# k-flouris/cmf

Hardware: AMD Instinct MI355X
Metric: log-density evals/sec (JtJ-cholesky path), MNIST D=784 d=64 bs=512 (higher is better)
Workload: dtype f32 (3x3 tangent convs as bf16x3 split MFMA, fp32 accumulate); 1 GPU; C3: MNIST-shaped (1,28,28) uint8-range + U[0,1) noise, non-square flow d=64, cholesky J^T J log-det + g_ij off-diagonal L1 + reconstruction, eval/no_grad; per_gpu_batch=512, global_batch=512, D=784, latent_dimension=64, parallelism=dp1

## Files before the change

### cmf_amd/_lib.py

```python
import ctypes as C
import os
import threading

_HERE = os.path.dirname(os.path.abspath(__file__))
LIB_PATH = os.path.join(_HERE, "libcmf_amd.so")

F_NONE, F_RELU, F_TANH, F_RAW, F_SELF_RELU, F_RELU_BITS = 0, 1, 2, 3, 4, 5
O_NONE, O_TANH, O_STANH = 0, 1, 2
GRAM_INVALID, GRAM_RING64, GRAM_DIRECT128, GRAM_WIDE, GRAM_RING_LIMIT = 0, 64, 128, 512, 0x7fffff00

_fp = C.c_void_p
_ll = C.c_longlong
_i = C.c_int
_f = C.c_float
_d = C.c_double


class ConvTangentArgs(C.Structure):
    _fields_ = [("x", _fp), ("x_np", _ll), ("x_ci", _ll), ("x_px", _ll),
                ("f", _fp), ("f_np", _ll), ("f_ci", _ll), ("f_px", _ll), ("fmode", _i),
                ("w", _fp),
                ("y", _fp), ("y_np", _ll), ("y_co", _ll), ("y_px", _ll),
                ("r", _fp), ("r_np", _ll), ("r_co", _ll), ("r_px", _ll),
                ("np", _i), ("cin", _i), ("cout", _i), ("H", _i), ("W", _i), ("nc", _i), ("taps", _i),
                ("bias", _fp), ("f_group", _i), ("x_sl", _ll), ("y_sl", _ll), ("r_sl", _ll),
                ("fo", _fp), ("fo_np", _ll), ("fo_co", _ll), ("fo_px", _ll), ("fomode", _i),
                ("mask_out", _fp), ("mask_np", _ll), ("amax_in", _fp), ("amax_out", _fp), ("live", _i),
                ("ymask", _fp), ("ymask_np", _ll),
                ("head_w", _fp), ("head_cout", _i), ("head_a", _fp), ("head_a_np", _ll), ("head_a_c", _ll), ("head_a_px", _ll),
                ("head_y", _fp), ("head_y_np", _ll), ("head_y_co", _ll), ("head_y_px", _ll),
                ("seed", _fp), ("seed_np", _ll), ("seed_col", _ll), ("seed_w", _fp),
                ("block_w1", _fp), ("block_m1", _fp), ("block_m1_np", _ll)]


class ConvPrimalArgs(C.Structure):
    _fields_ = [("x", _fp), ("x_b", _ll), ("x_c", _ll), ("x_px", _ll),
                ("f", _fp), ("f_c", _ll), ("f_px", _ll), ("imode", _i),
                ("w", _fp), ("bias", _fp), ("sw", _fp), ("sb", _fp),
                ("y", _fp), ("y_b", _ll), ("y_c", _ll), ("y_px", _ll),
                ("g", _fp),
                ("r", _fp), ("r_b", _ll), ("r_c", _ll), ("r_px", _ll),
                ("omode", _i),
                ("B", _i), ("cin", _i), ("cout", _i), ("H", _i), ("W", _i), ("taps", _i)]


class ProbeApplyArgs(C.Structure):
    _fields_ = [("r", _fp), ("r_np", _ll), ("r_px", _ll),
                ("t", _fp), ("t_np", _ll), ("t_c", _ll), ("t_px", _ll),
                ("cls", _fp),
                ("y", _fp), ("y_np", _ll), ("y_px", _ll),
                ("ymask", _fp), ("ymask_np", _ll),
                ("np", _i), ("cin", _i), ("H", _i), ("W", _i), ("nc", _i), ("ns", _i)]


MLP_MAX_LAYERS = 8
WGRAD_MAX_BATCH = 16


class MlpCouplerArgs(C.Structure):
    _fields_ = [("z", _fp), ("z_b", _ll), ("t", _fp), ("t_f", _ll), ("w", _fp),
                ("zi", _fp), ("si", _fp), ("ti", _fp), ("n_mod", _i),
                ("B", _i), ("cin", _i), ("chan_off", _i), ("chan_step", _i), ("n_layers", _i),
                ("width", _i * (MLP_MAX_LAYERS + 1)), ("w_off", _ll * MLP_MAX_LAYERS), ("decode", _i), ("lj", _fp), ("ncols", _i)]


SIGNATURES = {
    "cmf_version": (C.c_char_p, []),
    "cmf_pack_weight": (_i, [_fp, _fp, _i, _i, _i, _i, C.POINTER(_ll), _fp]),
    "cmf_pack_weights_batched": (_i, [_fp, _i, _fp]),
    "cmf_conv_tangent": (_i, [C.POINTER(ConvTangentArgs), _fp]),
    "cmf_pack_weight_bf16x3": (_i, [_fp, _fp, _i, _i, C.POINTER(_ll), _fp]),
    "cmf_pack_weight_bf16x3_t": (_i, [_fp, _fp, _i, _i, _i, C.POINTER(_ll), _fp]),
    "cmf_conv_tangent_bf16x3": (_i, [C.POINTER(ConvTangentArgs), _fp]),
    "cmf_probe_apply": (_i, [C.POINTER(ProbeApplyArgs), _fp]),
    "cmf_pack_seed_weight": (_i, [_fp, _fp, _fp]),
    "cmf_seed_panel": (_i, [_fp, _ll, _ll, _fp, _fp, _ll, _ll, _i, _i, _i, _i, _fp]),
    "cmf_pack_block_weight": (_i, [_fp, _fp, C.POINTER(_ll), _fp]),
    "cmf_pack_weight_f16x3": (_i, [_fp, _fp, _i, _i, _i, C.POINTER(_ll), _fp]),
    "cmf_conv_tangent_f16x3": (_i, [C.POINTER(ConvTangentArgs), _fp]),
    "cmf_conv_tangent_f16x3_item": (_i, [C.POINTER(ConvTangentArgs), _i, _fp]),
    "cmf_absmax": (_i, [_fp, _ll, _fp, _fp]),
    "cmf_conv_tangent_wgrad_ws": (_ll, [C.POINTER(ConvTangentArgs)]),
    "cmf_conv_tangent_wgrad": (_i, [C.POINTER(ConvTangentArgs), _fp, _fp, _fp, _ll, _fp]),
    "cmf_conv_tangent_wgrad_bf16x3": (_i, [C.POINTER(ConvTangentArgs), _fp, _fp, _fp, _ll, _fp]),
    "cmf_conv_tangent_wgrad_bf16x3_batched": (_i, [C.POINTER(ConvTangentArgs), _i, C.POINTER(_fp), C.POINTER(_fp), C.POINTER(_fp), _fp, _ll, _fp]),
    "cmf_primal_regroup": (_i, [_fp, _fp, _i, _ll, _i, _fp]),
    "cmf_conv_primal": (_i, [C.POINTER(ConvPrimalArgs), _fp]),
    "cmf_acl_primal": (_i, [_fp, _ll, _fp, _ll, _fp, _fp, _fp, _i, _i, _i, _fp, _fp]),
    "cmf_acl_tangent": (_i, [_fp, _ll, _ll, _fp, _ll, _ll, _i, _fp, _ll, _fp, _ll, _fp, _fp, _fp, _fp, _i, _i, _fp]),
    "cmf_acl_cotangent": (_i, [_fp, _ll, _ll, _fp, _ll, _ll, _i, _fp, _ll, _fp, _ll, _fp, _fp, _fp, _fp, _i, _i, _fp]),
    "cmf_acl_primal_backward": (_i, [_fp, _ll, _fp, _ll, _fp, _ll, _fp, _fp, _fp, _fp, _i, _i, _i, _fp, _fp]),
    "cmf_acl_cross_terms": (_i, [_fp, _ll, _ll, _fp, _ll, _ll, _fp, _ll, _ll, _i, _fp, _ll, _fp, _ll, _fp, _fp, _fp, _fp, _i, _i,
                            _fp, _fp, _fp, _fp]),
    "cmf_gather_primal": (_i, [_fp, _ll, _fp, _ll, _fp, _i, _i, _fp]),
    "cmf_gather_tangent": (_i, [_fp, _ll, _ll, _fp, _ll, _ll, _fp, _i, _i, _i, _fp]),
    "cmf_seed_tangent": (_i, [_fp, _ll, _ll, _fp, _i, _i, _fp, _i, _i, _i, _fp]),
    "cmf_gram_cholesky": (_i, [_fp, _ll, _ll, _i, _i, _i, _i, _fp, _fp, _fp, _fp, _fp, _fp, _fp]),
    "cmf_cholesky_retry": (_i, [_fp, _i, _i, _i, _f, _fp, _fp, _fp, _fp, _fp]),
    "cmf_gram_cholesky_family": (_i, [_i, _i, _ll]),
    "cmf_gram_condition": (_i, [_fp, _fp, _i, _i, _f, _fp, _fp, _fp, _fp, _fp]),
    "cmf_metric_stats_ws": (_ll, [_i, _i, _i, _i]),
    "cmf_metric_stats_accumulate": (_i, [_fp, _i, _i, _i, _fp, _fp, _ll, _fp, _fp]),
    "cmf_gram_spectrum": (_i, [_fp, _i, _i, _fp, _fp, _fp, _fp, _fp]),
    "cmf_gauss_newton_step": (_i, [_fp, _ll, _ll, _i, _i, _i, _i, _fp, _fp, _fp, _fp, _fp, _fp, _fp, _fp, _fp]),
    "cmf_weighted_gauss_newton_step": (_i, [_fp, _ll, _ll, _i, _i, _i, _i, _fp, _fp, _fp, _fp, _fp, _fp, _fp, _fp, _fp, _fp]),
    "cmf_operator_apply": (_i, [_fp, _i, _i, _fp, _ll, _ll, _i, _i, _fp, _fp, _ll, _ll, _fp, _fp]),
    "cmf_cross_gram": (_i, [_fp, _ll, _ll, _i, _i, _i, _i, _i, _fp, _fp]),
    "cmf_curve_step_ws": (_ll, [_i, _i, _i]),
    "cmf_curve_step": (_i, [_fp, _ll, _ll, _i, _i, _i, _i, _i, _fp, _fp, _fp, _fp, _fp, _fp, _fp, _fp, _fp, _fp, _ll, _fp]),
    "cmf_metric_solve": (_i, [_fp, _fp, _i, _i, _i, _fp, _fp, _fp, _fp, _fp]),
# ... 133 lines not shown
```

### cmf_amd/csrc/conv_block_head.hip

```cpp
#include <stdint.h>

#include "common.h"

namespace {

typedef __bf16 bf16x8 __attribute__((ext_vector_type(8)));
typedef __bf16 bf16x2 __attribute__((ext_vector_type(2)));
typedef float f32x2 __attribute__((ext_vector_type(2)));
typedef unsigned u32x4 __attribute__((ext_vector_type(4)));

constexpr int HID = 64, KJ = HID * 9, NT = 512, ROWS = 16, ND = 25, HALO = 8, XB = 4;
constexpr int SLICE = HID * 16;
static_assert(2 * KJ > 2 * NT && 2 * KJ <= 3 * NT && (2 * KJ - 2 * NT) % 64 == 0, "phase B: two units per thread, a third for whole waves");
constexpr int W1_FRAGS = 9 * 4 * 2 * 2 * 64;

__device__ __forceinline__ unsigned pack_hi(float a, float b, float& ra, float& rb) {
  bf16x2 h = __builtin_convertvector(f32x2{a, b}, bf16x2);
  const unsigned bits = __builtin_bit_cast(unsigned, h);
  ra = a - __builtin_bit_cast(float, bits << 16);
  rb = b - __builtin_bit_cast(float, bits & 0xffff0000u);
  return bits;
}
__device__ __forceinline__ unsigned pack_lo(float a, float b) {
  bf16x2 h = __builtin_convertvector(f32x2{a, b}, bf16x2);
  return __builtin_bit_cast(unsigned, h);
}

__global__ void pack_block_weight_kernel(const float* __restrict__ w, u32x4* __restrict__ out) {
  const int idx = blockIdx.x * 256 + threadIdx.x;
  if (idx >= W1_FRAGS) return;
  const int l = idx & 63, hl = (idx >> 6) & 1, ks = (idx >> 7) & 1, ct = (idx >> 8) & 3, t1 = idx >> 10;
  const int c = 16 * ct + (l & 15), ci0 = 32 * ks + 8 * (l >> 4);
  unsigned r[4];
#pragma unroll
  for (int jj = 0; jj < 4; ++jj) {
    const float v0 = w[((ci0 + 2 * jj) * HID + c) * 9 + t1], v1 = w[((ci0 + 2 * jj + 1) * HID + c) * 9 + t1];
    float ra, rb;
    const unsigned h = pack_hi(v0, v1, ra, rb);
    r[jj] = hl ? pack_lo(ra, rb) : h;
  }
  out[idx] = u32x4{r[0], r[1], r[2], r[3]};
}

struct Tile {
  int row0, s0, xb, Ws, H, W, live;
  __device__ __forceinline__ bool slot(int p, int& row, int& col, int& po) const {
    const int s = s0 + (p & 1);
    row = row0 + (p >> 1);
    col = live ? 2 * s + ((row + live - 1) & 1) : s;
    po = row * Ws + s;
    return row < H && s < Ws;
  }
};

__device__ __forceinline__ void load_w1(u32x4 (&b)[2][2], const u32x4* __restrict__ wp, int ct, int lane, int t1) {
#pragma unroll
  for (int ks = 0; ks < 2; ++ks)
#pragma unroll
    for (int hl = 0; hl < 2; ++hl) b[ks][hl] = wp[(((t1 * 4 + ct) * 2 + ks) * 2 + hl) * 64 + lane];
}

template <int HALF, int CP>
__device__ __forceinline__ void build_half(const u32x4* __restrict__ wp, const u32x4* As, float* Ks, const float* Gs,
                                           const unsigned long long* ha, const int* ctr, int ct, int lane) {
  constexpr int D0 = HALF ? 12 : 0, NDH = HALF ? 13 : 12;
  const f32x4 zero = {0.f, 0.f, 0.f, 0.f};
  f32x4 acc[NDH];
  u32x4 af[9][2][2], bw[2][2][2];
#pragma unroll
  for (int i = 0; i < NDH; ++i) acc[i] = zero;
  load_w1(bw[0], wp, ct, lane, 0);
#pragma unroll
  for (int t2 = 0; t2 < 9; ++t2)
#pragma unroll
    for (int ks = 0; ks < 2; ++ks)
#pragma unroll
      for (int hl = 0; hl < 2; ++hl) af[t2][ks][hl] = As[((t2 * 2 + ks) * 2 + hl) * 64 + lane];
#pragma unroll
  for (int t1 = 0; t1 < 9; ++t1) {
    if (t1 < 8) load_w1(bw[(t1 + 1) & 1], wp, ct, lane, t1 + 1);
#pragma unroll
    for (int t2 = 0; t2 < 9; ++t2) {
      const int d = (t1 / 3 + t2 / 3) * 5 + t1 % 3 + t2 % 3;
      if (d >= D0 && d < D0 + NDH) {
#pragma unroll
        for (int ks = 0; ks < 2; ++ks) {
          const bf16x8 ah = __builtin_bit_cast(bf16x8, af[t2][ks][0]), al = __builtin_bit_cast(bf16x8, af[t2][ks][1]);
          const bf16x8 bh = __builtin_bit_cast(bf16x8, bw[t1 & 1][ks][0]), bl = __builtin_bit_cast(bf16x8, bw[t1 & 1][ks][1]);
          acc[d - D0] = __builtin_amdgcn_mfma_f32_16x16x32_bf16(al, bh, acc[d - D0], 0, 0, 0);
          acc[d - D0] = __builtin_amdgcn_mfma_f32_16x16x32_bf16(ah, bl, acc[d - D0], 0, 0, 0);
          acc[d - D0] = __builtin_amdgcn_mfma_f32_16x16x32_bf16(ah, bh, acc[d - D0], 0, 0, 0);
        }
// ... 233 lines not shown
          if (o < cout && (N >= 16 || !(lane & 4))) yb[(long long)o * a.head_y_co + (idx & 3)] = val[i];
        }
      }
    }
  }
}

template <int CP>
int launch(const cmf_conv_tangent_args& a, hipStream_t s) {
  constexpr int P = ROWS / CP, TR = P / 2;
  const int Ws = a.live ? a.W / 2 : a.W;
  const long long tiles_x = (Ws + 1) / 2, tiles = tiles_x * ((a.H + TR - 1) / TR), ntiles = tiles * a.np;
  if (ntiles > 0x7ffffff0LL) return CMF_ERANGE;
  const int grid = 8 * (int)((ntiles + 7) / 8);
  hipLaunchKernelGGL(conv_block_head_kernel<CP>, dim3(grid), dim3(NT), 0, s, a, (int)tiles_x, (int)tiles, (int)ntiles);
  CMF_LAUNCH_CHECK();
  return 0;
}

}

extern "C" int cmf_pack_block_weight(const float* w, void* out, long long* out_bytes, void* stream) {
  if (!out) {
    if (!out_bytes) return CMF_EINVAL;
    *out_bytes = (long long)W1_FRAGS * 16;
    return 0;
  }
  if (!w || (uintptr_t)out % 16 || (uintptr_t)w % 4) return CMF_EINVAL;
  hipLaunchKernelGGL(pack_block_weight_kernel, dim3((W1_FRAGS + 255) / 256), dim3(256), 0, (hipStream_t)stream, w, (u32x4*)out);
  CMF_LAUNCH_CHECK();
  return 0;
}

int cmf_conv_block_head(const cmf_conv_tangent_args& a, hipStream_t s) {
  if (!a.x || !a.w || !a.f || !a.block_w1 || !a.block_m1 || !a.head_w || !a.head_a || !a.head_y) return CMF_EINVAL;
  if (a.r && a.r != a.x) return CMF_EINVAL;
  if (a.fmode != CMF_F_RELU_BITS || a.taps != 9 || a.cin != HID || a.cout != HID) return CMF_EINVAL;
  if (a.head_cout < 1 || a.head_cout > 8 || a.np <= 0 || a.H <= 0 || a.W <= 0 || a.nc <= 0 || a.nc % 16) return CMF_EINVAL;
  if (a.bias || a.fo || a.ymask || a.mask_out || a.seed || a.live < 0 || a.live > 2 || (a.live && a.W % 2)) return CMF_EINVAL;
  if (!((a.W % 14 == 0 && a.H % 2 == 0) || (a.W % 8 == 0 && a.H % 4 == 0))) return CMF_EINVAL;
  const long long HW = (long long)a.H * a.W;
  if (HW > (1 << 24)) return CMF_ERANGE;
  if (a.x_ci != 16 || a.x_sl != SLICE) return CMF_EINVAL;
  if ((a.x_np | a.x_px | a.head_y_np | a.head_y_co | a.head_y_px) % 4) return CMF_EINVAL;
  if (a.x_px < (long long)HID * a.nc || a.head_y_px < a.nc) return CMF_EINVAL;
  if ((uintptr_t)a.x % 16 || (uintptr_t)a.head_y % 16 || (uintptr_t)a.w % 4 || (uintptr_t)a.head_w % 4 || (uintptr_t)a.block_w1 % 16)
    return CMF_EINVAL;
  if ((uintptr_t)a.f % 8 || a.f_np % 8 || a.f_np < HW * (HID / 8)) return CMF_EINVAL;
  if ((uintptr_t)a.block_m1 % 8 || a.block_m1_np % 8 || a.block_m1_np < HW * (HID / 8)) return CMF_EINVAL;
  const int cp = a.head_cout <= 2 ? 2 : a.head_cout <= 4 ? 4 : 8;
  return cp == 2 ? launch<2>(a, s) : cp == 4 ? launch<4>(a, s) : launch<8>(a, s);
}
```

### cmf_amd/engine.py

```python
import ctypes as C
import threading
from typing import NamedTuple

import numpy as np
import torch
import torch.nn as nn

from . import _lib
from ._lib import (F_NONE, F_RELU, F_TANH, F_RAW, F_SELF_RELU, F_RELU_BITS, O_NONE, O_TANH, O_STANH, ConvPrimalArgs,
                   ConvTangentArgs)


def _stream():
    return C.c_void_p(torch.cuda.current_stream().cuda_stream)


def _p(t):
    return None if t is None else C.c_void_p(t.data_ptr())


def require_gpu(t, what="input"):
    if not t.is_cuda:
        raise RuntimeError(f"cmf_amd: {what} is on {t.device}; the log-density path runs only through the HIP "
                           "kernels on an AMD GPU (there is no CPU fallback)")
# ... 360 lines not shown
        run = launch

        def launch():
            with _lib.role("primal"):
                run()

    def cost():
        px_in = float(H) * W * nc * np_
        px = px_in * (0.5 if live else 1.0)
        return (2.0 * (cin + (1 if seed is not None else 0)) * cout * taps * px,
                4.0 * (px_in * cin + px * (cout + (cout if res_t is not None else 0))
                       + (float(seed["np"]) * np_ if seed is not None else 0.0)))
    return _timed(f"conv_tangent_t{taps}_ci{cin}_co{cout}" + ("_primal" if fmode == F_SELF_RELU else "_primal_bwd" if pbwd else "_live" if live else ""),
                  cost, launch)


def _conv_tangent_head(lib, a, x_t, x_off, x_np, x_ci, x_px, weight, taps, y_t, y_np, y_co, y_px, np_, cin, cout, H, W, nc, fmode, f,
                       f_np, res_t, res_off, res_np, x_sl, y_off, live, head):
    wf, act = head["weight"], head["act"]
    hc = int(wf.shape[0])
    w2, wf = weight.detach(), wf.detach().reshape(hc, -1)
    assert w2.is_contiguous() and wf.is_contiguous() and act.is_contiguous() and w2.dtype == wf.dtype == act.dtype == torch.float32
    a.x = C.c_void_p(x_t.data_ptr() + 4 * int(x_off)); a.x_np, a.x_ci, a.x_px, a.x_sl = int(x_np), int(x_ci), int(x_px), int(x_sl)
    a.f = _p(f); a.f_np = int(f_np); a.fmode = int(fmode)
    a.w = _p(w2)
    a.r = None if res_t is None else C.c_void_p(res_t.data_ptr() + 4 * int(res_off))
    a.r_np, a.r_co, a.r_px, a.r_sl = int(x_np if res_np is None else res_np), int(x_ci), int(x_px), int(x_sl)
    a.np, a.cin, a.cout, a.H, a.W, a.nc, a.taps, a.live = int(np_), int(cin), int(cout), int(H), int(W), int(nc), int(taps), int(live)
    blk = head.get("conv1")
    if blk is not None:
        assert res_t is None and isinstance(blk["mask"], BitMask), "the folded block reads h as x and takes relu'(c1) from a BitMask"
        a.block_w1 = _p(_block_pack(blk["weight"], x_t.device))
        a.block_m1, a.block_m1_np = _p(blk["mask"].data), int(blk["mask"].np_bytes)
    a.head_w, a.head_cout = _p(wf), hc
    a.head_a = _p(act); a.head_a_np, a.head_a_c, a.head_a_px = int(cin) * H * W, H * W, 1
    a.head_y = C.c_void_p(y_t.data_ptr() + 4 * int(y_off)); a.head_y_np, a.head_y_co, a.head_y_px = int(y_np), int(y_co), int(y_px)
    launch = lambda: _lib.check(lib.cmf_conv_tangent_bf16x3(C.byref(a), _stream()), "cmf_conv_tangent_bf16x3")

    def cost():
        px_out = float(H) * W * np_ * (0.5 if live else 1.0)
        if blk is not None:
            return (2.0 * hc * px_out * (cin * taps * cout + 3 * taps * cin * taps * cout + 25 * cout * nc),
                    4.0 * (float(H) * W * np_ * (nc * cin + 4) + px_out * (cout + nc * hc)))
        return (2.0 * hc * px_out * (cin * taps * cout + (cin * taps + cout) * nc),
                4.0 * (float(H) * W * np_ * nc * cin + px_out * (nc * cout + cout + nc * hc)))
    return _timed(f"conv_tangent_t{taps}_ci{cin}_co{cout}" + ("_live" if live else ""), cost, launch)


_WGRAD_WS = {}


def conv_tangent_wgrad(x_t, x_off, x_np, x_ci, x_px, gy_t, gy_off, y_np, y_co, y_px, dw, taps, np_, cin, cout, H, W, nc,
                       fmode=F_NONE, f=None, f_np=0, f_ci=0, f_px=0, f_group=1, x_sl=16, y_sl=16, precision=None):
    lib = _lib.load()
    assert dw.dtype == torch.float32 and dw.is_contiguous() and dw.numel() == cout * cin * taps
    a = ConvTangentArgs()
    a.x = C.c_void_p(x_t.data_ptr() + 4 * int(x_off)); a.x_np, a.x_ci, a.x_px = int(x_np), int(x_ci), int(x_px)
    fbits = isinstance(f, BitMask)
    if fbits:
        f, f_np, f_ci, f_px, fmode = f.data, f.np_bytes, 0, 0, F_RELU_BITS
    a.f = _p(f); a.f_np, a.f_ci, a.f_px = int(f_np), int(f_ci), int(f_px); a.fmode = fmode
    a.y_np, a.y_co, a.y_px = int(y_np), int(y_co), int(y_px)
    a.np, a.cin, a.cout, a.H, a.W, a.nc, a.taps = int(np_), int(cin), int(cout), int(H), int(W), int(nc), int(taps)
    a.f_group = int(f_group)
    a.x_sl, a.y_sl = int(x_sl), int(y_sl)
    need = int(lib.cmf_conv_tangent_wgrad_ws(C.byref(a)))
    key = (x_t.device, torch.cuda.current_stream().cuda_stream)
    ws = _WGRAD_WS.get(key)
    if ws is None or ws.numel() * 4 < need:
        ws = _WGRAD_WS[key] = torch.empty(need // 4, dtype=torch.float32, device=x_t.device)
# ... 1317 lines not shown
    y = primal_regroup(yg.view(G, -1), False).view(B, cout, H, W)
    g = primal_regroup(gg.view(G, -1), False).view(B, cout, H, W)
    if not need_acts:
        return y, g, None
    std_of = lambda t: primal_regroup(t.view(G, -1), False).view(B, hid, H, W)
    if train:
        out = ActList([a0] + masks[:-1] + [std_of(acts[-1])] if bits else [a0] + [std_of(t) for t in acts[1:]])
        out.grouped = acts
        return y, g, out
    if bits:
        return y, g, [a0] + masks[:-1] + [std_of(acts[-1])]
    return y, g, [a0] + [std_of(t) for t in acts[1:]]


def _view_rows(T, view):
    if T.layout == "panel":
        HW = view.geom.HW
        rows = T.data[: T.B * T.N * T.nc].view(T.B, T.N // HW, HW * T.nc)[:, view.chan_off::view.chan_step][:, :view.cin]
        out = Tangent(T.B, view.cin * HW, T.nc, "panel", T.data.device)
    else:
        rows = T.data[: T.B * T.N * T.nc].view(T.N, T.B * T.nc)[view.chan_off::view.chan_step][:view.cin]
        out = Tangent(T.B, view.cin, T.nc, "fmajor", T.data.device)
    out.data.view(rows.shape).copy_(rows)
    return out


CHECKERBOARD_TAIL = True
SKIP_DEAD_ROWS = True
FOLD_HEAD = True
FOLD_BLOCK = True
PROBE_FRONT = True
SEED_RESIDUAL = True
FOLD_BLOCK_SHAPES = ((28, 28, 2),)
PROBE_FRONT_SHAPES = {(28, 28, 1)}
PROBE_CLASSES = 13


def probe_plan(mask):
    mask = np.asarray(mask)
    if mask.ndim != 3:
        return None
    cin, H, W = mask.shape
    if not 1 <= cin <= 2:
        return None
    r, col = np.meshgrid(np.arange(H), np.arange(W), indexing="ij")
    cls = (np.mod(r - 5 * col, 2 * PROBE_CLASSES) >> 1)[None] + PROBE_CLASSES * np.arange(cin)[:, None, None]
    cls = np.where(mask != 0, cls, -1).astype(np.int8)
    for r0 in range(H):
        for c0 in range(W):
            win = cls[:, max(r0 - 2, 0):r0 + 3, max(c0 - 2, 0):c0 + 3].reshape(-1)
            win = win[win >= 0]
            if len(np.unique(win)) != len(win):
                return None
    ns = (PROBE_CLASSES * cin + 15) // 16
    flat = cls.reshape(-1)
    probes = np.zeros((cin * H * W, 16 * ns), dtype=np.float32)
    rows = np.flatnonzero(flat >= 0)
    probes[rows, flat[rows]] = 1.0
    return {"cls": flat, "ns": ns, "probes": probes}


def probe_apply(R, r_np, r_px, T, t_off, t_np, t_c, t_px, cls, y, y_np, y_px, np_, cin, H, W, nc, ns, ymask=None):
    a = _lib.ProbeApplyArgs()
    a.r = _p(R); a.r_np, a.r_px = int(r_np), int(r_px)
    a.t = C.c_void_p(T.data_ptr() + 4 * int(t_off)); a.t_np, a.t_c, a.t_px = int(t_np), int(t_c), int(t_px)
    a.cls = _p(cls)
# ... 32 lines not shown
            out[:, 16 * kq:16 * kq + 16, j] = w[:, 3 * kq + j].reshape(4, 16)
    return out


def seed_panel_index(H, W):
    idx = np.full(seed_plane(H, W), -1, dtype=np.int64)
    r, c = np.meshgrid(np.arange(H), np.arange(W), indexing="ij")
    idx[((r + 1) * (W + 2) + c + 1).reshape(-1)] = (r * W + c).reshape(-1)
    return idx


def _seed_pack(conv0, dev):
    def build():
        w = conv0.weight.detach().contiguous()
        assert tuple(w.shape) == (64, 1, 3, 3) and w.dtype == torch.float32
        out = torch.empty(4096, dtype=torch.uint8, device=dev)
        _lib.check(_lib.load().cmf_pack_seed_weight(_p(w), _p(out), _stream()), "cmf_pack_seed_weight")
        return out

    return DERIVED.get((id(conv0.weight), "seed-residual", str(dev)), [conv0.weight], build)


def _block_pack(weight, dev):
    def build():
        w = weight.detach().contiguous()
        assert tuple(w.shape) == (64, 64, 3, 3) and w.dtype == torch.float32
        n = C.c_longlong(0)
        _lib.check(_lib.load().cmf_pack_block_weight(None, None, C.byref(n), None), "pack size")
        out = torch.empty(n.value, dtype=torch.uint8, device=dev)
        _lib.check(_lib.load().cmf_pack_block_weight(_p(w), _p(out), None, _stream()), "cmf_pack_block_weight")
        return out

    return DERIVED.get((id(weight), "fold-block", str(dev)), [weight], build)


def _probe_hidden(conv0, view, plan, H, W, hid, dev):
    HW, ncp = H * W, 16 * plan["ns"]

    def build():
        out = torch.empty(HW * hid * ncp, dtype=torch.float32, device=dev)
        conv_tangent(plan["probes"], 0, view.cin * HW * ncp, HW * ncp, ncp, conv0.weight, 9, out, hid * HW * ncp, 16, hid * ncp,
                     1, view.cin, hid, H, W, ncp, fmode=F_RAW, f=view.mask, f_np=0, f_ci=HW, f_px=1, y_sl=hid * 16)
        return out

    return DERIVED.get((id(conv0.weight), "probe-front", H, W, view.cin, str(dev)), [conv0.weight], build)


def probe_front(conv0, conv1, T, view, plan, factor, ymask, scratch, u, H, W):
    B, nc, HW, hid, dev = T.B, T.nc, H * W, conv1.out_channels, T.data.device
    assert hid == 64 and T.layout == "panel"
    ncp = 16 * plan["ns"]
    conv_tangent(_probe_hidden(conv0, view, plan, H, W, hid, dev), 0, 0, 16, hid * ncp, conv1.weight, 9, scratch,
                 hid * HW * ncp, 16, hid * ncp, B, hid, hid, H, W, ncp, x_sl=hid * 16, y_sl=hid * 16, ymask=ymask, **factor)
    probe_apply(scratch, hid * HW * ncp, hid * ncp, T.data, view.chan_off * HW * nc, T.t_b, view.chan_step * HW * nc, nc,
                plan["cls"], u, hid * HW * nc, hid * nc, B, view.cin, H, W, nc, plan["ns"], ymask=ymask)


class TangentPlan(NamedTuple):
    filt: bool
    front: str
    tail: str
    compact: bool


def resnet_tangent_plan(net, view, nc, layout, acts, training):
    conv0, blocks, convf = _resnet_parts(net)
# ... 340 lines not shown
```

### include/cmf_amd.h

```cpp
#ifndef CMF_AMD_H
#define CMF_AMD_H

#ifdef __cplusplus
extern "C" {
#endif

#define CMF_EINVAL (-1)
#define CMF_ERANGE (-2)

#define CMF_F_NONE 0
#define CMF_F_RELU 1
#define CMF_F_TANH 2
#define CMF_F_RAW  3
#define CMF_F_SELF_RELU 4
#define CMF_F_RELU_BITS 5

#define CMF_O_NONE  0
#define CMF_O_TANH  1
#define CMF_O_STANH 2

const char* cmf_version(void);

int cmf_pack_weight(const float* w, float* out, int cout, int cin, int taps, int transpose,
                    long long* out_floats, void* stream);

typedef struct {
  const float* w; void* out; long long total;
  int cout, cin, taps, transpose, kind, reserved;
} cmf_pack_desc;
int cmf_pack_weights_batched(const cmf_pack_desc* table, int n, void* stream);

typedef struct {
  const float* x; long long x_np, x_ci, x_px;
  const float* f; long long f_np, f_ci, f_px;
  int fmode;
  const float* w;
  float* y;       long long y_np, y_co, y_px;
  const float* r; long long r_np, r_co, r_px;
  int np, cin, cout, H, W, nc, taps;
  const float* bias;
  int f_group;
  long long x_sl, y_sl, r_sl;
  const float* fo; long long fo_np, fo_co, fo_px; int fomode;
  void* mask_out; long long mask_np;
  const float* amax_in; float* amax_out;
  int live;
  const void* ymask; long long ymask_np;
  const float* head_w; int head_cout;
  const float* head_a; long long head_a_np, head_a_c, head_a_px;
  float* head_y; long long head_y_np, head_y_co, head_y_px;
  const float* seed; long long seed_np, seed_col; const void* seed_w;
  const void* block_w1; const void* block_m1; long long block_m1_np;
} cmf_conv_tangent_args;
int cmf_conv_tangent(const cmf_conv_tangent_args* a, void* stream);

int cmf_pack_weight_bf16x3(const float* w, void* out, int cout, int cin, long long* out_bytes, void* stream);
int cmf_pack_weight_bf16x3_t(const float* w, void* out, int cout, int cin, int transpose, long long* out_bytes, void* stream);
int cmf_conv_tangent_bf16x3(const cmf_conv_tangent_args* a, void* stream);
int cmf_pack_seed_weight(const float* w, void* out, void* stream);
int cmf_pack_block_weight(const float* w, void* out, long long* out_bytes, void* stream);
int cmf_seed_panel(const float* v, long long v_np, long long v_px, const float* mask, float* out, long long out_np, long long out_col,
                   int np, int H, int W, int nc, void* stream);

typedef struct {
  const float* r; long long r_np, r_px;
  const float* t; long long t_np, t_c, t_px;
  const signed char* cls;
  float* y;       long long y_np, y_px;
  const void* ymask; long long ymask_np;
  int np, cin, H, W, nc, ns;
} cmf_probe_apply_args;
int cmf_probe_apply(const cmf_probe_apply_args* a, void* stream);

int cmf_pack_weight_f16x3(const float* w, void* out, int cout, int cin, int transpose, long long* out_bytes, void* stream);
int cmf_conv_tangent_f16x3(const cmf_conv_tangent_args* a, void* stream);
int cmf_conv_tangent_f16x3_item(const cmf_conv_tangent_args* a, int item_channels, void* stream);
int cmf_absmax(const float* x, long long n, float* out, void* stream);

long long cmf_conv_tangent_wgrad_ws(const cmf_conv_tangent_args* a);
int cmf_conv_tangent_wgrad(const cmf_conv_tangent_args* a, const float* gy, float* dw, float* ws, long long ws_bytes,
                           void* stream);
int cmf_conv_tangent_wgrad_bf16x3(const cmf_conv_tangent_args* a, const float* gy, float* dw, float* ws, long long ws_bytes,
                                  void* stream);
#define CMF_WGRAD_MAX_BATCH 16
int cmf_conv_tangent_wgrad_bf16x3_batched(const cmf_conv_tangent_args* a, int nprob, const float* const* x, const float* const* gy,
                                          float* const* dw, float* ws, long long ws_bytes, void* stream);

typedef struct {
  const float* x; long long x_b, x_c, x_px;
  const float* f; long long f_c, f_px;
  int imode;
  const float* w; const float* bias;
  const float* sw; const float* sb;
// ... 168 lines not shown
```

Measured before the change: 1558 evals/s.

## Split folded conv block-head into build and apply kernels via workspace

The fused block-head kernel is split in two. A build kernel computes the per-tile folded 5x5 kernel K (E = W2·G, masked, then convolved with W1 through bf16x3 MFMA) and writes it to a global workspace. An apply kernel then streams the hidden activations against K across channel-slice groups in a second grid dimension. This separates the heavy per-tile kernel construction from the per-slice apply, so each gets its own block size and occupancy and the apply can parallelise over slices. The cost is an extra global round trip for K, a second launch and a cached workspace allocation. It is enabled by default for the 28x28, head_cout=2 shape.

```diff
diff --git a/cmf_amd/_lib.py b/cmf_amd/_lib.py
--- a/cmf_amd/_lib.py
+++ b/cmf_amd/_lib.py
@@ -30,7 +30,8 @@
                 ("head_w", _fp), ("head_cout", _i), ("head_a", _fp), ("head_a_np", _ll), ("head_a_c", _ll), ("head_a_px", _ll),
                 ("head_y", _fp), ("head_y_np", _ll), ("head_y_co", _ll), ("head_y_px", _ll),
                 ("seed", _fp), ("seed_np", _ll), ("seed_col", _ll), ("seed_w", _fp),
-                ("block_w1", _fp), ("block_m1", _fp), ("block_m1_np", _ll)]
+                ("block_w1", _fp), ("block_m1", _fp), ("block_m1_np", _ll),
+                ("block_k", _fp), ("block_k_bytes", _ll)]
 
 
 class ConvPrimalArgs(C.Structure):
@@ -76,6 +77,8 @@
     "cmf_pack_seed_weight": (_i, [_fp, _fp, _fp]),
     "cmf_seed_panel": (_i, [_fp, _ll, _ll, _fp, _fp, _ll, _ll, _i, _i, _i, _i, _fp]),
     "cmf_pack_block_weight": (_i, [_fp, _fp, C.POINTER(_ll), _fp]),
+    "cmf_conv_block_workspace": (_i, [C.POINTER(ConvTangentArgs), C.POINTER(_ll)]),
+    "cmf_conv_block_phase": (_i, [C.POINTER(ConvTangentArgs), _i, _fp]),
     "cmf_pack_weight_f16x3": (_i, [_fp, _fp, _i, _i, _i, C.POINTER(_ll), _fp]),
     "cmf_conv_tangent_f16x3": (_i, [C.POINTER(ConvTangentArgs), _fp]),
     "cmf_conv_tangent_f16x3_item": (_i, [C.POINTER(ConvTangentArgs), _i, _fp]),
diff --git a/cmf_amd/csrc/conv_block.h b/cmf_amd/csrc/conv_block.h
--- /dev/null
+++ b/cmf_amd/csrc/conv_block.h
@@ -0,0 +1,56 @@
+#pragma once
+#include <stdint.h>
+
+#include "common.h"
+
+namespace cmf_block {
+
+typedef __bf16 bf16x8 __attribute__((ext_vector_type(8)));
+typedef __bf16 bf16x2 __attribute__((ext_vector_type(2)));
+typedef float f32x2 __attribute__((ext_vector_type(2)));
+typedef unsigned u32x4 __attribute__((ext_vector_type(4)));
+
+constexpr int HID = 64, KJ = HID * 9, ROWS = 16, ND = 25, HALO = 8, XB = 4;
+constexpr int SLICE = HID * 16;
+constexpr int W1_FRAGS = 9 * 4 * 2 * 2 * 64;
+constexpr int A_FRAGS = 9 * 2 * 2 * 64;
+constexpr int K_CHUNK = ROWS * ND * 16, K_TILE = 4 * K_CHUNK;
+
+__device__ __forceinline__ unsigned pack_hi(float a, float b, float& ra, float& rb) {
+  bf16x2 h = __builtin_convertvector(f32x2{a, b}, bf16x2);
+  const unsigned bits = __builtin_bit_cast(unsigned, h);
+  ra = a - __builtin_bit_cast(float, bits << 16);
+  rb = b - __builtin_bit_cast(float, bits & 0xffff0000u);
+  return bits;
+}
+__device__ __forceinline__ unsigned pack_lo(float a, float b) {
+  bf16x2 h = __builtin_convertvector(f32x2{a, b}, bf16x2);
+  return __builtin_bit_cast(unsigned, h);
+}
+
+struct Tile {
+  int row0, s0, xb, Ws, H, W, live;
+  __device__ __forceinline__ bool slot(int p, int& row, int& col, int& po) const {
+    const int s = s0 + (p & 1);
+    row = row0 + (p >> 1);
+    col = live ? 2 * s + ((row + live - 1) & 1) : s;
+    po = row * Ws + s;
+    return row < H && s < Ws;
+  }
+};
+
+__device__ __forceinline__ void load_w1(u32x4 (&b)[2][2], const u32x4* __restrict__ wp, int ct, int lane, int t1) {
+#pragma unroll
+  for (int ks = 0; ks < 2; ++ks)
+#pragma unroll
+    for (int hl = 0; hl < 2; ++hl) b[ks][hl] = wp[(((t1 * 4 + ct) * 2 + ks) * 2 + hl) * 64 + lane];
+}
+
+static inline void tile_counts(const cmf_conv_tangent_args& a, int cp, long long& tiles_x, long long& tiles, long long& ntiles) {
+  const int P = ROWS / cp, TR = P / 2, Ws = a.live ? a.W / 2 : a.W;
+  tiles_x = (Ws + 1) / 2, tiles = tiles_x * ((a.H + TR - 1) / TR), ntiles = tiles * a.np;
+}
+
+}
+
+int cmf_conv_block_split(const cmf_conv_tangent_args& a, int cp, int phases, hipStream_t s);
diff --git a/cmf_amd/csrc/conv_block_head.hip b/cmf_amd/csrc/conv_block_head.hip
--- a/cmf_amd/csrc/conv_block_head.hip
+++ b/cmf_amd/csrc/conv_block_head.hip
@@ -1,30 +1,11 @@
-#include <stdint.h>
-
-#include "common.h"
+#include "conv_block.h"
 
 namespace {
 
-typedef __bf16 bf16x8 __attribute__((ext_vector_type(8)));
-typedef __bf16 bf16x2 __attribute__((ext_vector_type(2)));
-typedef float f32x2 __attribute__((ext_vector_type(2)));
-typedef unsigned u32x4 __attribute__((ext_vector_type(4)));
-
-constexpr int HID = 64, KJ = HID * 9, NT = 512, ROWS = 16, ND = 25, HALO = 8, XB = 4;
-constexpr int SLICE = HID * 16;
+using namespace cmf_block;
+
+constexpr int NT = 512;
 static_assert(2 * KJ > 2 * NT && 2 * KJ <= 3 * NT && (2 * KJ - 2 * NT) % 64 == 0, "phase B: two units per thread, a third for whole waves");
-constexpr int W1_FRAGS = 9 * 4 * 2 * 2 * 64;
-
-__device__ __forceinline__ unsigned pack_hi(float a, float b, float& ra, float& rb) {
-  bf16x2 h = __builtin_convertvector(f32x2{a, b}, bf16x2);
-  const unsigned bits = __builtin_bit_cast(unsigned, h);
-  ra = a - __builtin_bit_cast(float, bits << 16);
-  rb = b - __builtin_bit_cast(float, bits & 0xffff0000u);
-  return bits;
-}
-__device__ __forceinline__ unsigned pack_lo(float a, float b) {
-  bf16x2 h = __builtin_convertvector(f32x2{a, b}, bf16x2);
-  return __builtin_bit_cast(unsigned, h);
-}
 
 __global__ void pack_block_weight_kernel(const float* __restrict__ w, u32x4* __restrict__ out) {
   const int idx = blockIdx.x * 256 + threadIdx.x;
@@ -40,24 +21,6 @@
     r[jj] = hl ? pack_lo(ra, rb) : h;
   }
   out[idx] = u32x4{r[0], r[1], r[2], r[3]};
-}
-
-struct Tile {
-  int row0, s0, xb, Ws, H, W, live;
-  __device__ __forceinline__ bool slot(int p, int& row, int& col, int& po) const {
-    const int s = s0 + (p & 1);
-    row = row0 + (p >> 1);
-    col = live ? 2 * s + ((row + live - 1) & 1) : s;
-    po = row * Ws + s;
-    return row < H && s < Ws;
-  }
-};
-
-__device__ __forceinline__ void load_w1(u32x4 (&b)[2][2], const u32x4* __restrict__ wp, int ct, int lane, int t1) {
-#pragma unroll
-  for (int ks = 0; ks < 2; ++ks)
-#pragma unroll
-    for (int hl = 0; hl < 2; ++hl) b[ks][hl] = wp[(((t1 * 4 + ct) * 2 + ks) * 2 + hl) * 64 + lane];
 }
 
 template <int HALF, int CP>
@@ -357,7 +320,7 @@
   return 0;
 }
 
-int cmf_conv_block_head(const cmf_conv_tangent_args& a, hipStream_t s) {
+static int check_block(const cmf_conv_tangent_args& a, int& cp) {
   if (!a.x || !a.w || !a.f || !a.block_w1 || !a.block_m1 || !a.head_w || !a.head_a || !a.head_y) return CMF_EINVAL;
   if (a.r && a.r != a.x) return CMF_EINVAL;
   if (a.fmode != CMF_F_RELU_BITS || a.taps != 9 || a.cin != HID || a.cout != HID) return CMF_EINVAL;
@@ -373,6 +336,43 @@
     return CMF_EINVAL;
   if ((uintptr_t)a.f % 8 || a.f_np % 8 || a.f_np < HW * (HID / 8)) return CMF_EINVAL;
   if ((uintptr_t)a.block_m1 % 8 || a.block_m1_np % 8 || a.block_m1_np < HW * (HID / 8)) return CMF_EINVAL;
-  const int cp = a.head_cout <= 2 ? 2 : a.head_cout <= 4 ? 4 : 8;
+  cp = a.head_cout <= 2 ? 2 : a.head_cout <= 4 ? 4 : 8;
+  return 0;
+}
+
+static long long workspace_bytes(const cmf_conv_tangent_args& a, int cp) {
+  long long tiles_x, tiles, ntiles;
+  tile_counts(a, cp, tiles_x, tiles, ntiles);
+  return ntiles * K_TILE * (long long)sizeof(float);
+}
+
+static int check_workspace(const cmf_conv_tangent_args& a, int cp) {
+  if (!a.block_k || (uintptr_t)a.block_k % 16 || a.block_k_bytes < workspace_bytes(a, cp)) return CMF_EINVAL;
+  return 0;
+}
+
+extern "C" int cmf_conv_block_workspace(const cmf_conv_tangent_args* a, long long* out_bytes) {
+  if (!a || !out_bytes || a->head_cout < 1 || a->head_cout > 8 || a->np <= 0 || a->H <= 0 || a->W <= 0 || a->live < 0 || a->live > 2 ||
+      (a->live && a->W % 2))
+    return CMF_EINVAL;
+  *out_bytes = workspace_bytes(*a, a->head_cout <= 2 ? 2 : a->head_cout <= 4 ? 4 : 8);
+  return 0;
+}
+
+extern "C" int cmf_conv_block_phase(const cmf_conv_tangent_args* a, int phases, void* stream) {
+  int cp = 0;
+  if (!a || phases < 1 || phases > 3) return CMF_EINVAL;
+  if (int e = check_block(*a, cp)) return e;
+  if (int e = check_workspace(*a, cp)) return e;
+  return cmf_conv_block_split(*a, cp, phases, (hipStream_t)stream);
+}
+
+int cmf_conv_block_head(const cmf_conv_tangent_args& a, hipStream_t s) {
+  int cp = 0;
+  if (int e = check_block(a, cp)) return e;
+  if (a.block_k || a.block_k_bytes) {
+    if (int e = check_workspace(a, cp)) return e;
+    return cmf_conv_block_split(a, cp, 3, s);
+  }
   return cp == 2 ? launch<2>(a, s) : cp == 4 ? launch<4>(a, s) : launch<8>(a, s);
 }
diff --git a/cmf_amd/csrc/conv_block_split.hip b/cmf_amd/csrc/conv_block_split.hip
--- /dev/null
+++ b/cmf_amd/csrc/conv_block_split.hip
@@ -0,0 +1,411 @@
+#include "conv_block.h"
+
+namespace {
+
+using namespace cmf_block;
+
+constexpr int BT = 256;
+static_assert(KJ > 2 * BT && KJ <= 3 * BT && KJ - 2 * BT == 64, "build, E: two pairs per thread, a third for wave 0");
+static_assert(K_CHUNK % 4 == 0, "16-byte pieces");
+
+__device__ __forceinline__ int item_of(int n) {
+  const int per = (n + 7) >> 3;
+  return (int)(blockIdx.x & 7) * per + (int)(blockIdx.x >> 3);
+}
+
+__device__ __forceinline__ Tile tile_of(const cmf_conv_tangent_args& a, int tl, int tiles_x, int TR) {
+  const int ty = tl / tiles_x, tx = tl - ty * tiles_x;
+  Tile T;
+  T.H = a.H, T.W = a.W, T.live = a.live, T.Ws = a.live ? a.W >> 1 : a.W, T.row0 = ty * TR, T.s0 = 2 * tx, T.xb = a.live ? 4 * tx : 2 * tx;
+  return T;
+}
+
+__device__ __forceinline__ unsigned long long mask_word(const void* m, long long np_bytes, int b, int px) {
+  return *reinterpret_cast<const unsigned long long*>(reinterpret_cast<const unsigned char*>(m) + (long long)b * np_bytes + (long long)px * (HID / 8));
+}
+
+
+template <int R>
+__device__ __forceinline__ void build_e(float (&acc)[3][2 * ROWS], const float* __restrict__ w2, const float* Gs, int tid) {
+#pragma unroll
+  for (int r = 0; r < R; ++r)
+#pragma unroll
+    for (int i = 0; i < 2 * ROWS; ++i) acc[r][i] = 0.f;
+#pragma unroll 4
+  for (int c = 0; c < HID; ++c) {
+    float w[R];
+#pragma unroll
+    for (int r = 0; r < R; ++r) w[r] = w2[c * KJ + tid + r * BT];
+#pragma unroll
+    for (int i4 = 0; i4 < 2 * ROWS / 4; ++i4) {
+      const f32x4 g = *reinterpret_cast<const f32x4*>(&Gs[c * 2 * ROWS + 4 * i4]);
+#pragma unroll
+      for (int r = 0; r < R; ++r)
+#pragma unroll
+        for (int k = 0; k < 4; ++k) acc[r][4 * i4 + k] = fmaf(g[k], w[r], acc[r][4 * i4 + k]);
+    }
+  }
+}
+
+template <int R, int CP>
+__device__ __forceinline__ void store_e(const float (&acc)[3][2 * ROWS], const unsigned long long* um, unsigned short* A16, int tid) {
+  constexpr int P = ROWS / CP;
+#pragma unroll
+  for (int r = 0; r < R; ++r) {
+    const int q = tid + r * BT, ci = q / 9, tap = q - ci * 9, ks = ci >> 5, kq = (ci >> 3) & 3, j = ci & 7;
+#pragma unroll
+    for (int i = 0; i < 2 * ROWS; i += 2) {
+      const int t = i >> 4, row = i & 15;
+      const float e0 = ((um[(t * P + row / CP) * 9 + tap] >> ci) & 1) ? acc[r][i] : 0.f;
+      const float e1 = ((um[(t * P + (row + 1) / CP) * 9 + tap] >> ci) & 1) ? acc[r][i + 1] : 0.f;
+      float ra, rb;
+      const unsigned h = pack_hi(e0, e1, ra, rb);
+      const unsigned l = pack_lo(ra, rb);
+      const int at = t * (A_FRAGS * 8) + ((tap * 2 + ks) * 2 * 64 + kq * 16 + row) * 8 + j;
+      A16[at] = (unsigned short)(h & 0xffffu);
+      A16[at + 8] = (unsigned short)(h >> 16);
+      A16[at + 64 * 8] = (unsigned short)(l & 0xffffu);
+      A16[at + 64 * 8 + 8] = (unsigned short)(l >> 16);
+    }
+  }
+}
+
+template <int HALF, int CP>
+__device__ __forceinline__ void build_k(const cmf_conv_tangent_args& a, const u32x4* __restrict__ wp, const u32x4* As, const unsigned long long* ha,
+                                        const unsigned long long* alv, const int* ctr, float* __restrict__ kt0, bool has1, int ct, int lane) {
+  constexpr int D0 = HALF ? 12 : 0, NDH = HALF ? 13 : 12, P = ROWS / CP, VW = CP < 4 ? CP : 4;
+  typedef float vecw __attribute__((ext_vector_type(VW)));
+  const f32x4 zero = {0.f, 0.f, 0.f, 0.f};
+  f32x4 acc[2][NDH];
+  u32x4 bw[2][2][2];
+#pragma unroll
+  for (int t = 0; t < 2; ++t)
+#pragma unroll
+    for (int i = 0; i < NDH; ++i) acc[t][i] = zero;
+  load_w1(bw[0], wp, ct, lane, 0);
+#pragma unroll
+  for (int t1 = 0; t1 < 9; ++t1) {
+    if (t1 < 8) load_w1(bw[(t1 + 1) & 1], wp, ct, lane, t1 + 1);
+    int al = lane;
+    asm volatile("" : "+v"(al));
+#pragma unroll
+    for (int t2 = 0; t2 < 9; ++t2) {
+      const int d = (t1 / 3 + t2 / 3) * 5 + t1 % 3 + t2 % 3;
+      if (d >= D0 && d < D0 + NDH) {
+#pragma unroll
+        for (int ks = 0; ks < 2; ++ks) {
+          const bf16x8 bh = __builtin_bit_cast(bf16x8, bw[t1 & 1][ks][0]), bl = __builtin_bit_cast(bf16x8, bw[t1 & 1][ks][1]);
+#pragma unroll
+          for (int t = 0; t < 2; ++t) {
+            const bf16x8 ah = __builtin_bit_cast(bf16x8, As[t * A_FRAGS + ((t2 * 2 + ks) * 2 + 0) * 64 + al]);
+            const bf16x8 alo = __builtin_bit_cast(bf16x8, As[t * A_FRAGS + ((t2 * 2 + ks) * 2 + 1) * 64 + al]);
+            acc[t][d - D0] = __builtin_amdgcn_mfma_f32_16x16x32_bf16(alo, bh, acc[t][d - D0], 0, 0, 0);
+            acc[t][d - D0] = __builtin_amdgcn_mfma_f32_16x16x32_bf16(ah, bl, acc[t][d - D0], 0, 0, 0);
+            acc[t][d - D0] = __builtin_amdgcn_mfma_f32_16x16x32_bf16(ah, bh, acc[t][d - D0], 0, 0, 0);
+          }
+        }
+      }
+    }
+  }
+  const int c = 16 * ct + (lane & 15);
+#pragma unroll
+  for (int t = 0; t < 2; ++t) {
+    if (t && !has1) break;
+    float* kt = kt0 + (long long)t * K_TILE + ct * K_CHUNK + (lane & 15) * CP;
+#pragma unroll
+    for (int dl = 0; dl < NDH; ++dl) {
+      const int d = D0 + dl;
+#pragma unroll
+      for (int i0 = 0; i0 < 4; i0 += VW) {
+        const int row = 4 * (lane >> 4) + i0, p = row / CP, o0 = row % CP;
+        const int at = ctr[t * P + p];
+        const bool on = at >= 0 && ((ha[t * HALO * HALO + (at >= 0 ? at + (d / 5 - 2) * HALO + d % 5 - 2 : 0)] >> c) & 1);
+        vecw v;
+#pragma unroll
+        for (int i = 0; i < VW; ++i) {
+          v[i] = on ? acc[t][dl][i0 + i] : 0.f;
+          if (d == 12) {
+            const int o = o0 + i;
+            const float g = (((alv[t * P + p] >> c) & 1) && o < a.head_cout) ? a.head_w[o * HID + c] : 0.f;
+            v[i] = g + v[i];
+          }
+        }
+        *reinterpret_cast<vecw*>(kt + (p * ND + d) * 16 * CP + o0) = v;
+      }
+    }
+  }
+}
+
+template <int CP>
+__global__ __launch_bounds__(BT, 2) void conv_block_build_kernel(cmf_conv_tangent_args a, int tiles_x, int tiles_per_sample, int ntiles) {
+  constexpr int P = ROWS / CP, TR = P / 2;
+  static_assert(P >= 2, "two output columns per tile");
+  __shared__ __attribute__((aligned(16))) u32x4 As[2 * A_FRAGS];
+  __shared__ unsigned long long um[2 * P * 9];
+  __shared__ unsigned long long ha[2 * HALO * HALO];
+  __shared__ unsigned long long alv[2 * P];
+  __shared__ int ctr[2 * P];
+  float* Gs = reinterpret_cast<float*>(As);
+
+  const int item = item_of((ntiles + 1) >> 1);
+  if (2 * item >= ntiles) return;
+  const int tid = threadIdx.x, lane = tid & 63, wv = __builtin_amdgcn_readfirstlane(tid >> 6);
+  const int H = a.H, W = a.W, cout = a.head_cout;
+  const bool has1 = 2 * item + 1 < ntiles;
+
+  for (int u = tid; u < 2 * P * 9; u += BT) {
+    const int t = u / (P * 9), p = (u - t * P * 9) / 9, tap = u % 9, tg = 2 * item + t;
+    unsigned long long m = 0;
+    if (tg < ntiles) {
+      const int b = tg / tiles_per_sample;
+      const Tile T = tile_of(a, tg - b * tiles_per_sample, tiles_x, TR);
+      int row, col, po;
+      if (T.slot(p, row, col, po)) {
+        const int r = row + tap / 3 - 1, c = col + tap % 3 - 1;
+        if (r >= 0 && r < H && c >= 0 && c < W) m = mask_word(a.block_m1, a.block_m1_np, b, r * W + c);
+      }
+    }
+    um[u] = m;
+  }
+  if (tid >= 128) {
+    const int t = (tid - 128) >> 6, q = tid & 63, tg = 2 * item + t;
+    unsigned long long m = 0;
+    if (tg < ntiles) {
+      const int b = tg / tiles_per_sample;
+      const Tile T = tile_of(a, tg - b * tiles_per_sample, tiles_x, TR);
+      const int r = T.row0 - 2 + (q >> 3), c = T.xb - 2 + (q & 7);
+      if (r >= 0 && r < H && c >= 0 && c < W) m = mask_word(a.f, a.f_np, b, r * W + c);
+    }
+    ha[t * HALO * HALO + q] = m;
+  }
+  for (int pp = wv; pp < 2 * P; pp += BT / 64) {
+    const int t = pp / P, p = pp - t * P, tg = 2 * item + t;
+    int row = 0, col = 0, po, b = 0;
+    bool ok = false;
+    Tile T = tile_of(a, 0, tiles_x, TR);
+    if (tg < ntiles) {
+      b = tg / tiles_per_sample;
+      T = tile_of(a, tg - b * tiles_per_sample, tiles_x, TR);
+      ok = T.slot(p, row, col, po);
+    }
+    bool on = false;
+    if (ok) on = a.head_a[(long long)b * a.head_a_np + (long long)lane * a.head_a_c + (long long)(row * W + col) * a.head_a_px] > 0.f;
+    const unsigned long long bal = __ballot(on);
+    if (lane == 0) {
+      alv[pp] = bal;
+      ctr[pp] = ok ? (row - (T.row0 - 2)) * HALO + (col - (T.xb - 2)) : -1;
+    }
+#pragma unroll
+    for (int o = 0; o < CP; ++o) Gs[lane * 2 * ROWS + t * ROWS + p * CP + o] = (on && o < cout) ? a.head_w[o * HID + lane] : 0.f;
+  }
+  __syncthreads();
+
+  float e[3][2 * ROWS];
+  if (wv == 0)
+    build_e<3>(e, a.w, Gs, tid);
+  else
+    build_e<2>(e, a.w, Gs, tid);
+  __syncthreads();
+  if (wv == 0)
+    store_e<3, CP>(e, um, reinterpret_cast<unsigned short*>(As), tid);
+  else
+    store_e<2, CP>(e, um, reinterpret_cast<unsigned short*>(As), tid);
+  __syncthreads();
+
+  const u32x4* wp = reinterpret_cast<const u32x4*>(a.block_w1);
+  float* kt0 = reinterpret_cast<float*>(a.block_k) + (long long)(2 * item) * K_TILE;
+  build_k<0, CP>(a, wp, As, ha, alv, ctr, kt0, has1, wv, lane);
+  build_k<1, CP>(a, wp, As, ha, alv, ctr, kt0, has1, wv, lane);
+}
+
+
+template <int CP>
+__global__ __launch_bounds__(BT, 3) void conv_block_apply_kernel(cmf_conv_tangent_args a, int tiles_x, int tiles_per_sample, int ntiles) {
+  constexpr int P = ROWS / CP, TR = P / 2, NQ = P >= 4 ? 4 : 2, PU = P / NQ, NS = NQ, NV = K_CHUNK / 4, NL = (NV + BT - 1) / BT;
+  __shared__ __attribute__((aligned(16))) float Kb[2][K_CHUNK];
+  __shared__ unsigned long long hl[HALO * HALO];
+  __shared__ unsigned long long alv[P];
+  __shared__ int ctr[P];
+
+  const int item = item_of(ntiles);
+  if (item >= ntiles) return;
+  const int b = item / tiles_per_sample;
+  const int tid = threadIdx.x, lane = tid & 63, wv = __builtin_amdgcn_readfirstlane(tid >> 6);
+  const int H = a.H, W = a.W, cout = a.head_cout;
+  const Tile T = tile_of(a, item - b * tiles_per_sample, tiles_x, TR);
+  const int y0 = T.row0 - 2, x0 = T.xb - 2;
+
+  const f32x4* kg = reinterpret_cast<const f32x4*>(a.block_k) + (long long)item * (K_TILE / 4);
+  f32x4 kr[NL];
+#pragma unroll
+  for (int i = 0; i < NL; ++i)
+    if (tid + i * BT < NV) kr[i] = kg[tid + i * BT];
+
+  if (tid < HALO * HALO) {
+    const int r = y0 + (tid >> 3), c = x0 + (tid & 7);
+    hl[tid] = (r >= 0 && r < H && c >= 0 && c < W) ? mask_word(a.f, a.f_np, b, r * W + c) : 0ull;
+  }
+  for (int p = wv; p < P; p += BT / 64) {
+    int row, col, po;
+    const bool ok = T.slot(p, row, col, po);
+    bool on = false;
+    if (ok) on = a.head_a[(long long)b * a.head_a_np + (long long)lane * a.head_a_c + (long long)(row * W + col) * a.head_a_px] > 0.f;
+    const unsigned long long bal = __ballot(on);
+    if (lane == 0) {
+      alv[p] = bal;
+      ctr[p] = ok ? (row - y0) * HALO + (col - x0) : -1;
+    }
+  }
+  __syncthreads();
+  if (tid < P && ctr[tid] >= 0) hl[ctr[tid]] |= alv[tid];
+#pragma unroll
+  for (int i = 0; i < NL; ++i)
+    if (tid + i * BT < NV) reinterpret_cast<f32x4*>(Kb[0])[tid + i * BT] = kr[i];
+  __syncthreads();
+
+  const int nsl = a.nc >> 4, cl = lane >> 2, ph = wv % NQ;
+  int prow[PU], pcol[PU], ppo[PU], sl[NS];
+  bool pok[PU], sok[NS];
+  int ylo = H, yhi = -1, xlo = W, xhi = -1;
+#pragma unroll
+  for (int k = 0; k < PU; ++k) {
+    pok[k] = T.slot(ph * PU + k, prow[k], pcol[k], ppo[k]);
+    if (pok[k]) {
+      ylo = min(ylo, prow[k] - 2), yhi = max(yhi, prow[k] + 2);
+      xlo = min(xlo, pcol[k] - 2), xhi = max(xhi, pcol[k] + 2);
+    }
+  }
+  ylo = max(ylo, 0), yhi = min(yhi, H - 1), xlo = max(xlo, 0), xhi = min(xhi, W - 1);
+#pragma unroll
+  for (int j = 0; j < NS; ++j) {
+    sl[j] = (int)blockIdx.y * 4 + wv / NQ + (4 / NQ) * j;
+    sok[j] = sl[j] < nsl;
+  }
+  if (!sok[0]) yhi = -1;
+  const float* hb = a.x + (long long)b * a.x_np + lane * 4;
+  const f32x4 zero = {0.f, 0.f, 0.f, 0.f};
+  f32x4 acc[NS][PU][CP];
+#pragma unroll
+  for (int j = 0; j < NS; ++j)
+#pragma unroll
+    for (int k = 0; k < PU; ++k)
+#pragma unroll
+      for (int o = 0; o < CP; ++o) acc[j][k][o] = zero;
+
+#pragma unroll 1
+  for (int ch = 0; ch < 4; ++ch) {
+    const float* Kc = Kb[ch & 1];
+    for (int y = ylo; y <= yhi; ++y) {
+#pragma unroll 1
+      for (int xs = xlo; xs <= xhi; xs += XB) {
+        f32x4 v[XB][NS];
+#pragma unroll
+        for (int xi = 0; xi < XB; ++xi) {
+#pragma unroll
+          for (int j = 0; j < NS; ++j) v[xi][j] = zero;
+          const int x = xs + xi;
+          if (x <= xhi) {
+            const unsigned long long m = hl[(y - y0) * HALO + (x - x0)];
+            if ((m >> (ch * 16 + cl)) & 1) {
+              const float* src = hb + (long long)(y * W + x) * a.x_px + ch * 256;
+#pragma unroll
+              for (int j = 0; j < NS; ++j)
+                if (sok[j]) v[xi][j] = *reinterpret_cast<const f32x4*>(src + sl[j] * SLICE);
+            }
+          }
+        }
+#pragma unroll
+        for (int xi = 0; xi < XB; ++xi) {
+          const int x = xs + xi;
+#pragma unroll
+          for (int k = 0; k < PU; ++k) {
+            const int dy = y - prow[k] + 2, dx = x - pcol[k] + 2;
+            if (x <= xhi && pok[k] && dy >= 0 && dy < 5 && dx >= 0 && dx < 5) {
+              const float* e4 = static_cast<const float*>(
+                  __builtin_assume_aligned(&Kc[(((ph * PU + k) * ND + dy * 5 + dx) * 16 + cl) * CP], CP < 4 ? 8 : 16));
+#pragma unroll
+              for (int o = 0; o < CP; ++o) {
+                const float e = e4[o];
+#pragma unroll
+                for (int j = 0; j < NS; ++j)
+#pragma unroll
+                  for (int q = 0; q < 4; ++q) acc[j][k][o][q] = fmaf(e, v[xi][j][q], acc[j][k][o][q]);
+              }
+            }
+          }
+        }
+      }
+    }
+    if (ch < 3) {
+#pragma unroll
+      for (int i = 0; i < NL; ++i)
+        if (tid + i * BT < NV) kr[i] = kg[(ch + 1) * NV + tid + i * BT];
+#pragma unroll
+      for (int i = 0; i < NL; ++i)
+        if (tid + i * BT < NV) reinterpret_cast<f32x4*>(Kb[(ch + 1) & 1])[tid + i * BT] = kr[i];
+      __syncthreads();
+    }
+  }
+  if (yhi < 0) return;
+
+  constexpr int N = 4 * CP;
+#pragma unroll
+  for (int j = 0; j < NS; ++j) {
+    if (!sok[j]) continue;
+#pragma unroll
+    for (int k = 0; k < PU; ++k) {
+      float val[N];
+#pragma unroll
+      for (int o = 0; o < CP; ++o)
+#pragma unroll
+        for (int q = 0; q < 4; ++q) val[4 * o + q] = acc[j][k][o][q];
+#pragma unroll
+      for (int s = 0; s < 4; ++s) {
+        const int off = 32 >> s, n = N >> s;
+        if (n >= 2) {
+          const bool hi = lane & off;
+#pragma unroll
+          for (int i = 0; i < n / 2; ++i) {
+            const float mine = hi ? val[n / 2 + i] : val[i], send = hi ? val[i] : val[n / 2 + i];
+            val[i] = mine + __shfl_xor(send, off, 64);
+          }
+        } else {
+          val[0] += __shfl_xor(val[0], off, 64);
+        }
+      }
+      if (pok[k]) {
+        float* yb = a.head_y + (long long)b * a.head_y_np + (long long)ppo[k] * a.head_y_px + sl[j] * 16 + (lane & 3) * 4;
+        constexpr int KEEP = N >= 16 ? N / 16 : 1;
+#pragma unroll
+        for (int i = 0; i < KEEP; ++i) {
+          const int idx = ((cl * N) >> 4) + i, o = idx >> 2;
+          if (o < cout && (N >= 16 || !(lane & 4))) yb[(long long)o * a.head_y_co + (idx & 3)] = val[i];
+        }
+      }
+    }
+  }
+}
+
+template <int CP>
+int launch(const cmf_conv_tangent_args& a, int phases, hipStream_t s) {
+  long long tiles_x, tiles, ntiles;
+  tile_counts(a, CP, tiles_x, tiles, ntiles);
+  if (ntiles > 0x7ffffff0LL) return CMF_ERANGE;
+  if (phases & 1) {
+    const int grid = 8 * (int)(((ntiles + 1) / 2 + 7) / 8);
+    hipLaunchKernelGGL(conv_block_build_kernel<CP>, dim3(grid), dim3(BT), 0, s, a, (int)tiles_x, (int)tiles, (int)ntiles);
+    CMF_LAUNCH_CHECK();
+  }
+  if (phases & 2) {
+    const int grid = 8 * (int)((ntiles + 7) / 8), groups = ((a.nc >> 4) + 3) / 4;
+    hipLaunchKernelGGL(conv_block_apply_kernel<CP>, dim3(grid, groups), dim3(BT), 0, s, a, (int)tiles_x, (int)tiles, (int)ntiles);
+    CMF_LAUNCH_CHECK();
+  }
+  return 0;
+}
+
+}
+
+int cmf_conv_block_split(const cmf_conv_tangent_args& a, int cp, int phases, hipStream_t s) {
+  return cp == 2 ? launch<2>(a, phases, s) : cp == 4 ? launch<4>(a, phases, s) : launch<8>(a, phases, s);
+}
diff --git a/cmf_amd/engine.py b/cmf_amd/engine.py
--- a/cmf_amd/engine.py
+++ b/cmf_amd/engine.py
@@ -416,10 +416,18 @@
         assert res_t is None and isinstance(blk["mask"], BitMask), "the folded block reads h as x and takes relu'(c1) from a BitMask"
         a.block_w1 = _p(_block_pack(blk["weight"], x_t.device))
         a.block_m1, a.block_m1_np = _p(blk["mask"].data), int(blk["mask"].np_bytes)
+        a.head_cout = hc
+        split = blk.get("split")
+        if (FOLD_BLOCK_SPLIT and (int(H), int(W), hc) in FOLD_BLOCK_SPLIT_SHAPES) if split is None else split:
+            ws = blk.get("workspace")
+            ws = _block_workspace(a, x_t.device) if ws is None else ws
+            a.block_k, a.block_k_bytes = _p(ws), int(ws.numel() * ws.element_size())
     a.head_w, a.head_cout = _p(wf), hc
     a.head_a = _p(act); a.head_a_np, a.head_a_c, a.head_a_px = int(cin) * H * W, H * W, 1
     a.head_y = C.c_void_p(y_t.data_ptr() + 4 * int(y_off)); a.head_y_np, a.head_y_co, a.head_y_px = int(y_np), int(y_co), int(y_px)
     launch = lambda: _lib.check(lib.cmf_conv_tangent_bf16x3(C.byref(a), _stream()), "cmf_conv_tangent_bf16x3")
+    if blk is not None and blk.get("phases"):
+        launch = lambda: _lib.check(lib.cmf_conv_block_phase(C.byref(a), int(blk["phases"]), _stream()), "cmf_conv_block_phase")
 
     def cost():
         px_out = float(H) * W * np_ * (0.5 if live else 1.0)
@@ -1803,6 +1811,8 @@
 PROBE_FRONT = True
 SEED_RESIDUAL = True
 FOLD_BLOCK_SHAPES = ((28, 28, 2),)
+FOLD_BLOCK_SPLIT = True
+FOLD_BLOCK_SPLIT_SHAPES = ((28, 28, 2),)
 PROBE_FRONT_SHAPES = {(28, 28, 1)}
 PROBE_CLASSES = 13
 
@@ -1901,6 +1911,23 @@
         return out
 
     return DERIVED.get((id(weight), "fold-block", str(dev)), [weight], build)
+
+
+_BLOCK_WS = {}
+
+
+def block_workspace_bytes(a):
+    n = C.c_longlong(0)
+    _lib.check(_lib.load().cmf_conv_block_workspace(C.byref(a), C.byref(n)), "cmf_conv_block_workspace")
+    return int(n.value)
+
+
+def _block_workspace(a, dev):
+    need = block_workspace_bytes(a)
+    ws = _BLOCK_WS.get((dev, need))
+    if ws is None:
+        ws = _BLOCK_WS[(dev, need)] = torch.empty(need, dtype=torch.uint8, device=dev)
+    return ws
 
 
 def _probe_hidden(conv0, view, plan, H, W, hid, dev):
diff --git a/include/cmf_amd.h b/include/cmf_amd.h
--- a/include/cmf_amd.h
+++ b/include/cmf_amd.h
@@ -51,6 +51,7 @@
   float* head_y; long long head_y_np, head_y_co, head_y_px;
   const float* seed; long long seed_np, seed_col; const void* seed_w;
   const void* block_w1; const void* block_m1; long long block_m1_np;
+  void* block_k; long long block_k_bytes;
 } cmf_conv_tangent_args;
 int cmf_conv_tangent(const cmf_conv_tangent_args* a, void* stream);
 
@@ -59,6 +60,8 @@
 int cmf_conv_tangent_bf16x3(const cmf_conv_tangent_args* a, void* stream);
 int cmf_pack_seed_weight(const float* w, void* out, void* stream);
 int cmf_pack_block_weight(const float* w, void* out, long long* out_bytes, void* stream);
+int cmf_conv_block_workspace(const cmf_conv_tangent_args* a, long long* out_bytes);
+int cmf_conv_block_phase(const cmf_conv_tangent_args* a, int phases, void* stream);
 int cmf_seed_panel(const float* v, long long v_np, long long v_px, const float* mask, float* out, long long out_np, long long out_col,
                    int np, int H, int W, int nc, void* stream);
 
```

Measured after the change: 1562 evals/s (median of 6 runs). Within noise of the previous version (+0.2%).
